# qiskit-community/adapt-aqc

Hardware: AMD Instinct MI355X
Metric: overlap+gradient evals/sec, 50-qubit MPS chi=64, 1/2/4/8 MI355X (higher is better)
Workload: dtype c128

## Files before the change

### adaptaqc_amd/_lib.py

```python
import atexit
import ctypes
import os
import threading

import numpy as np

_HERE = os.path.dirname(os.path.abspath(__file__))
LIB_PATH = os.environ.get("AQC_LIB") or os.path.join(_HERE, "libaqchip.so")

OP_DTYPE = np.dtype(
    [("nq", "<i4"), ("q0", "<i4"), ("q1", "<i4"), ("flags", "<i4"), ("m", "<f8", (32,))], align=True
)
assert OP_DTYPE.itemsize == 272
OP_KRAUS1 = 1
OP_MEASURE1 = 2
OP_KRAUS2 = 3

EXPORTS = (
    "aqc_last_error", "aqc_version", "aqc_init", "aqc_finalize", "aqc_timing_enable",
    "aqc_timing_query", "aqc_timing_reset",
    "aqc_sv_create", "aqc_sv_destroy", "aqc_sv_reset", "aqc_sv_copy", "aqc_sv_apply", "aqc_sv_plan",
    "aqc_sv_amp0", "aqc_sv_z_all", "aqc_sv_get", "aqc_sv_set",
    "aqc_mps_create", "aqc_mps_destroy", "aqc_mps_set_truncation", "aqc_mps_set_vidal",
    "aqc_mps_get_vidal", "aqc_mps_get_dims", "aqc_mps_copy", "aqc_mps_copy_batch", "aqc_mps_apply",
    "aqc_mps_apply_batch", "aqc_mps_apply_sort_batch", "aqc_mps_apply_sort_batch_async", "aqc_mps_apply_batch_async", "aqc_mps_check_batch", "aqc_mps_sort", "aqc_mps_sort_batch", "aqc_mps_overlap_zero",
    "aqc_mps_overlap_zero_batch", "aqc_mps_dot", "aqc_mps_z_all", "aqc_mps_amps_hw1", "aqc_mps_z_all_batch", "aqc_mps_z_sum_batch", "aqc_mps_zero_hw1_batch",
    "aqc_mps_amps_hw1_batch",
    "aqc_pair_grads", "aqc_pair_grads_batch", "aqc_argmax_scaled", "aqc_argmax_scaled_batch", "aqc_mps_jacobi_stats",
    "aqc_mps_set_jacobi_tol", "aqc_mps_set_jacobi_stop", "aqc_mps_set_fused_chain", "aqc_mps_chain_ticks", "aqc_svd_debug",
    "aqc_sv_pair_rdms", "aqc_mps_pair_rdms", "aqc_mps_pair_rdms_batch", "aqc_entanglement_measures",
    "aqc_sv_transition", "aqc_mps_product_fit", "aqc_mps_set_svd_path", "aqc_svd_gram_ticks", "aqc_bj_ticks",
    "aqc_sweep_set_chain_mode", "aqc_stream_join", "aqc_stream_wait", "aqc_svd_gram_stats", "aqc_env_ticks",
    "aqc_comm_unique_id", "aqc_comm_init", "aqc_comm_destroy", "aqc_comm_rank", "aqc_allgather_f64",
    "aqc_allgather_f64_host", "aqc_allreduce_max_f64", "aqc_svd_gram_big_stats", "aqc_svd_gram_big_ticks",
    "aqc_gb_set_spin_limit", "aqc_gb_set_tail", "aqc_gb_set_stages", "aqc_debug_hog", "aqc_pool_stats",
    "aqc_scratch_stats", "aqc_mps_set_chain_epilogue", "aqc_mps_get_chain_epilogue", "aqc_mps_chain_epilogue_stats",
    "aqc_env_fallbacks", "aqc_env_set_single", "aqc_env_set_spin_limit",
    "aqc_sv_sample", "aqc_mps_sample", "aqc_sample_uniforms", "aqc_sv_traj_sample",
    "aqc_sv_traj_pair_tomo", "aqc_sv_traj_pauli_counts", "aqc_mps_traj_sample", "aqc_mps_traj_plan", "aqc_mps_traj_set_batch",
    "aqc_mps_traj_pair_tomo", "aqc_mps_traj_tomo_plan", "aqc_mps_traj_set_readout_batch",
    "aqc_sv_pauli_expect", "aqc_mps_pauli_expect", "aqc_mps_pauli_expect_batch",
    "aqc_pair_tomo_probs", "aqc_concurrence_bound_probs", "aqc_multinomial_counts", "aqc_tomo_fit",
)


class AqcError(RuntimeError):
    pass


_lock = threading.Lock()
_lib = None
_initialised_device = None

_P = ctypes.c_void_p
_I = ctypes.c_int
_D = ctypes.c_double
_DP = ctypes.POINTER(ctypes.c_double)
_IP = ctypes.POINTER(ctypes.c_int)

_SIGS = {
    "aqc_last_error": ([], ctypes.c_char_p),
    "aqc_version": ([], _I),
    "aqc_init": ([_I], _I),
    "aqc_finalize": ([], _I),
    "aqc_timing_enable": ([_I], _I),
    "aqc_timing_query": ([ctypes.c_char_p, _DP, ctypes.POINTER(ctypes.c_int64), _DP, _DP], _I),
    "aqc_timing_reset": ([], _I),
    "aqc_sv_create": ([_I, ctypes.POINTER(_P)], _I),
    "aqc_sv_destroy": ([_P], _I),
    "aqc_sv_reset": ([_P], _I),
    "aqc_sv_copy": ([_P, _P], _I),
    "aqc_sv_apply": ([_P, _P, _I], _I),
    "aqc_sv_plan": ([_I, _P, _I, _P], _I),
    "aqc_sv_amp0": ([_P, _DP, _DP], _I),
    "aqc_sv_z_all": ([_P, _DP], _I),
    "aqc_sv_get": ([_P, _P], _I),
    "aqc_sv_set": ([_P, _P], _I),
    "aqc_mps_create": ([_I, _I, _D, _I, ctypes.POINTER(_P)], _I),
    "aqc_mps_destroy": ([_P], _I),
    "aqc_mps_set_truncation": ([_P, _D, _I], _I),
    "aqc_mps_set_vidal": ([_P, _P, _P, _P], _I),
    "aqc_mps_get_vidal": ([_P, _P, _P, _P], _I),
    "aqc_mps_get_dims": ([_P, _P], _I),
    "aqc_mps_copy": ([_P, _P], _I),
    "aqc_mps_copy_batch": ([_P, _P, _I], _I),
    "aqc_mps_apply": ([_P, _P, _I], _I),
    "aqc_mps_apply_batch": ([_P, _I, _P, _P], _I),
    "aqc_mps_apply_sort_batch": ([_P, _I, _P, _P], _I),
    "aqc_mps_apply_sort_batch_async": ([_P, _I, _P, _P], _I),
    "aqc_mps_apply_batch_async": ([_P, _I, _P, _P], _I),
    "aqc_mps_check_batch": ([_P, _I], _I),
    "aqc_mps_sort": ([_P], _I),
    "aqc_mps_sort_batch": ([_P, _I], _I),
    "aqc_mps_overlap_zero": ([_P, _DP, _DP], _I),
    "aqc_mps_overlap_zero_batch": ([_P, _I, _P], _I),
    "aqc_mps_dot": ([_P, _P, _DP, _DP], _I),
    "aqc_mps_z_all": ([_P, _P], _I),
    "aqc_mps_amps_hw1": ([_P, _P], _I),
    "aqc_mps_z_all_batch": ([_P, _I, _P], _I),
    "aqc_mps_z_sum_batch": ([_P, _P, _I, _P], _I),
    "aqc_mps_zero_hw1_batch": ([_P, _P, _I, _P, _P], _I),
    "aqc_mps_amps_hw1_batch": ([_P, _I, _P], _I),
    "aqc_pair_grads": ([_P, _P, _P, _I, _P, _P, _P, _I, _P, _I], _I),
    "aqc_pair_grads_batch": ([_P, _I, _P, _P, _I, _P, _P, _P, _I, _P, _I], _I),
    "aqc_argmax_scaled": ([_P, _P, _I, _I, _IP], _I),
    "aqc_argmax_scaled_batch": ([_P, _I, _P, _I, _I, _P], _I),
    "aqc_mps_jacobi_stats": ([_P, _IP], _I),
    "aqc_mps_set_jacobi_tol": ([_D], _I),
    "aqc_mps_set_jacobi_stop": ([_D], _I),
    "aqc_mps_set_fused_chain": ([_I], _I),
    "aqc_mps_chain_ticks": ([_P], _I),
    "aqc_mps_set_chain_epilogue": ([_I], _I),
    "aqc_mps_get_chain_epilogue": ([], _I),
    "aqc_mps_chain_epilogue_stats": ([_P], _I),
    "aqc_svd_debug": ([_P, _I, _I, _I, _I, _P, _P, _P, _P], _I),
    "aqc_sv_pair_rdms": ([_P, _P, _I, _P], _I),
    "aqc_mps_pair_rdms": ([_P, _P, _I, _P], _I),
    "aqc_mps_pair_rdms_batch": ([_P, _I, _P, _I, _P, _I], _I),
    "aqc_entanglement_measures": ([_P, _I, _I, _P, _I], _I),
    "aqc_sv_transition": ([_P, _P, _I, _P], _I),
    "aqc_mps_product_fit": ([_P, _P, _I, _I, _I, _D, _DP, _IP], _I),
    "aqc_mps_set_svd_path": ([_I, _I], _I),
    "aqc_svd_gram_ticks": ([_P], _I),
    "aqc_bj_ticks": ([_P], _I),
    "aqc_sweep_set_chain_mode": ([_I], _I),
    "aqc_stream_join": ([_P], _I),
    "aqc_stream_wait": ([_P], _I),
    "aqc_svd_gram_stats": ([_P], _I),
    "aqc_env_ticks": ([_P], _I),
    "aqc_comm_unique_id": ([ctypes.c_char_p], _I),
    "aqc_comm_init": ([ctypes.c_char_p, _I, _I, ctypes.POINTER(_P)], _I),
    "aqc_comm_destroy": ([_P], _I),
    "aqc_comm_rank": ([_P, _IP, _IP], _I),
    "aqc_allgather_f64": ([_P, _P, _P, ctypes.c_size_t], _I),
    "aqc_allgather_f64_host": ([_P, _P, _P, ctypes.c_size_t], _I),
    "aqc_allreduce_max_f64": ([_P, _DP], _I),
    "aqc_svd_gram_big_stats": ([_P], _I),
    "aqc_svd_gram_big_ticks": ([_P], _I),
    "aqc_gb_set_spin_limit": ([_D], _I),
    "aqc_env_fallbacks": ([ctypes.POINTER(ctypes.c_longlong)], _I),
    "aqc_env_set_single": ([_I], _I),
    "aqc_env_set_spin_limit": ([_D], _I),
    "aqc_gb_set_tail": ([_I], _I),
    "aqc_gb_set_stages": ([_I], _I),
    "aqc_debug_hog": ([_I, _D], _I),
    "aqc_pool_stats": ([_P], _I),
    "aqc_scratch_stats": ([_P], _I),
    "aqc_sv_sample": ([_P, _I, ctypes.c_uint64, ctypes.c_uint64, _P, _P], _I),
    "aqc_mps_sample": ([_P, _I, ctypes.c_uint64, ctypes.c_uint64, _P, _P], _I),
    "aqc_sample_uniforms": ([ctypes.c_uint64, ctypes.c_uint64, _I, _I, _P], _I),
    "aqc_sv_traj_sample": ([_I, _P, _I, _I, ctypes.c_uint64, ctypes.c_uint64, _P, _P, _P], _I),
    "aqc_sv_traj_pair_tomo": ([_I, _P, _I, _P, _I, _P, _I, ctypes.c_uint64, ctypes.c_uint64, _P, _P, _P], _I),
    "aqc_sv_traj_pauli_counts": ([_I, _P, _I, _P, _I, _P, _I, ctypes.c_uint64, ctypes.c_uint64, _P, _P, _P, _P], _I),
    "aqc_mps_traj_sample": ([_I, _I, _D, _I, _P, _I, _I, ctypes.c_uint64, ctypes.c_uint64, _P, _P, _P], _I),
    "aqc_mps_traj_plan": ([_I, _P, _I, _P, _P, _I], _I),
    "aqc_mps_traj_set_batch": ([_I], _I),
    "aqc_mps_traj_pair_tomo": ([_I, _I, _D, _I, _P, _I, _P, _I, _P, _I, ctypes.c_uint64, ctypes.c_uint64, _P, _P, _P], _I),
    "aqc_mps_traj_tomo_plan": ([_I, _P, _I, _P, _P, _I], _I),
    "aqc_mps_traj_set_readout_batch": ([_I], _I),
    "aqc_sv_pauli_expect": ([_P, _P, _P, _I, _P], _I),
    "aqc_mps_pauli_expect": ([_P, _P, _I, _P], _I),
    "aqc_mps_pauli_expect_batch": ([_P, _I, _P, _I, _P], _I),
    "aqc_pair_tomo_probs": ([_P, _I, _P, _I], _I),
    "aqc_concurrence_bound_probs": ([_P, _I, _P, _I], _I),
    "aqc_multinomial_counts": ([_P, _I, _I, _I, ctypes.c_uint64, ctypes.c_uint64, _P, _P], _I),
    "aqc_tomo_fit": ([_P, _I, _P, _I], _I),
}


def load(path=LIB_PATH):
    global _lib
    with _lock:
        if _lib is not None:
            return _lib
        if not os.path.exists(path):
            raise AqcError(
                f"HIP library not found at {path}; build it with `python -c 'import __graft_entry__ as g; g.build()'`"
            )
        try:
            import torch
        except ImportError:
            pass
        lib = ctypes.CDLL(path)
        missing = []
        for name, (args, res) in _SIGS.items():
            f = getattr(lib, name, None)
            if f is None:
                missing.append(name)
                continue
            f.argtypes = args
            f.restype = res
        if missing and not os.environ.get("AQC_LIB"):
            raise AqcError(f"{path} lacks entry points {missing}: rebuild it (make -C adaptaqc_amd/csrc)")
        _lib = lib
        return lib

# ... 91 lines not shown
```

### adaptaqc_amd/csrc/mps.hip

```cpp
#include <algorithm>
#include <cmath>
#include <chrono>
#include <cstring>
#include <atomic>
#include <cstdlib>
#include <mutex>
#include <thread>
#include <unordered_set>

#include "aqc_gemm.h"
#include "mps_internal.h"

using aqc::cplx;

namespace aqc {

namespace {
std::mutex g_mps_stream_mu;
hipStream_t g_mps_streams[64] = {nullptr};
void release_mps_streams() {
  std::lock_guard<std::mutex> lk(g_mps_stream_mu);
  for (auto& s : g_mps_streams)
    if (s) (void)hipStreamDestroy(s), s = nullptr;
}
}

hipStream_t mps_stream() {
  int dev = 0;
  hipGetDevice(&dev);
  std::lock_guard<std::mutex> lk(g_mps_stream_mu);
  if (!g_mps_streams[dev]) {
    hipStreamCreateWithFlags(&g_mps_streams[dev], hipStreamNonBlocking);
    note_device(dev);
    on_finalize(release_mps_streams);
  }
  return g_mps_streams[dev];
}

hipStream_t mps_stream_if_any(int dev) {
  if (dev < 0 || dev >= 64) return nullptr;
  std::lock_guard<std::mutex> lk(g_mps_stream_mu);
  return g_mps_streams[dev];
}

StagingRing& staging_ring() {
  static PerDevice<StagingRing> rings;
  return rings.here();
}

}

namespace {

using aqc::fresh_tid;
using aqc::StagingLease;
using aqc::wave_sum_d;

constexpr int kT = 256;
constexpr double kChop = 1e-16;
constexpr int kMaxSweeps = 60;
double g_jacobi_tol_factor = 1.0;
constexpr double kDefaultTinyT = 1e-6;
constexpr double kStopCos = 3e-13;
constexpr int kStopCosSweeps = 30;
double g_jacobi_tiny_t = kDefaultTinyT;
constexpr double kJacobiNoise = 0.0;
bool g_fused_chain = true;
int g_chain_epilogue = [] {
  const char* e = std::getenv("AQC_CHAIN_EPILOGUE");
  const int v = e ? std::atoi(e) : 3;
  return v >= 0 && v <= 3 ? v : 3;
}();
int g_chain_min_states = 32;
constexpr int kChainLdsBytes = 4 * (int)sizeof(aqc::GemmLds);

struct OneSiteJob {
  cplx* g;
  const int* dims;
  int cap;
  int pad;
  cplx u[4];
};

using aqc::TwoSiteJob;
using aqc::kMaxCap;
using aqc::kSigMax;
using aqc::kSigTail;
using aqc::kSigLen;

__global__ void k_mps_zero(cplx* gam, double* lam, int* dims, int n, int cap) {
  const size_t ss = (size_t)2 * cap * cap;
  for (int i = blockIdx.x * blockDim.x + threadIdx.x; i < n; i += gridDim.x * blockDim.x) {
    gam[(size_t)i * ss] = aqc::cmk(1.0, 0.0);
  }
  for (int b = blockIdx.x * blockDim.x + threadIdx.x; b <= n; b += gridDim.x * blockDim.x) {
    lam[(size_t)b * cap] = 1.0;
    dims[b] = 1;
  }
}

__global__ __launch_bounds__(kT) void k_1q(const OneSiteJob* __restrict__ jobs) {
  const OneSiteJob& j = jobs[blockIdx.y];
  const int cl = j.dims[0], cr = j.dims[1];
  const int cap = j.cap;
  const size_t half = (size_t)cap * cap;
  for (int e = blockIdx.x * kT + threadIdx.x; e < cl * cr; e += gridDim.x * kT) {
    const int l = e / cr, r = e % cr;
    const size_t o = (size_t)l * cap + r;
    const cplx a0 = aqc::ldg(j.g + o), a1 = aqc::ldg(j.g + half + o);
    aqc::stg(j.g + o, aqc::cfma(j.u[1], a1, aqc::cmul(j.u[0], a0)));
    aqc::stg(j.g + half + o, aqc::cfma(j.u[3], a1, aqc::cmul(j.u[2], a0)));
  }
}

__global__ __launch_bounds__(kT) void k_theta(const TwoSiteJob* __restrict__ jobs, int nj) {
  int jb, tile;
  if (!aqc::xcd_job_block(nj, jb, tile)) return;
  const TwoSiteJob& j = jobs[jb];
  const int chl = j.dims[0], chm = j.dims[1], chr = j.dims[2];
  const int cap = j.cap;
  const int tiles_r = (cap + 15) / 16;
  const int l0 = (tile / tiles_r) * 16, r0 = (tile % tiles_r) * 16;
  if (l0 >= chl || r0 >= chr) return;
  __shared__ cplx As[2][16][17];
  __shared__ cplx Bs[2][16][17];
  const int ty = threadIdx.x / 16, tx = threadIdx.x % 16;
  const int l = l0 + ty, r = r0 + tx;
  const size_t half = (size_t)cap * cap;
  cplx acc[4];
#pragma unroll
  for (int i = 0; i < 4; ++i) acc[i] = aqc::cmk(0, 0);
  const double lll = l < chl ? j.ll[l] : 0.0;
  const double lrr = r < chr ? j.lr[r] : 0.0;
  for (int m0 = 0; m0 < chm; m0 += 16) {
    const int ma = m0 + tx, mb = m0 + ty;
#pragma unroll
    for (int s = 0; s < 2; ++s) {
      cplx a = aqc::cmk(0, 0), b = aqc::cmk(0, 0);
      if (l < chl && ma < chm) a = aqc::cscale(j.gp[s * half + (size_t)l * cap + ma], lll * j.lm[ma]);
      if (mb < chm && r < chr) b = aqc::cscale(j.gq[s * half + (size_t)mb * cap + r], lrr);
      As[s][ty][tx] = a;
      Bs[s][ty][tx] = b;
    }
    __syncthreads();
#pragma unroll 4
    for (int mm = 0; mm < 16; ++mm) {
      const cplx a0 = As[0][ty][mm], a1 = As[1][ty][mm];
      const cplx b0 = Bs[0][mm][tx], b1 = Bs[1][mm][tx];
      acc[0] = aqc::cfma(a0, b0, acc[0]);
      acc[1] = aqc::cfma(a0, b1, acc[1]);
      acc[2] = aqc::cfma(a1, b0, acc[2]);
      acc[3] = aqc::cfma(a1, b1, acc[3]);
    }
    __syncthreads();
// ... 806 lines not shown
  const double* llp = j.ll;
  const double* lmp = j.lm;
  const double* lrp = j.lr;
  asm volatile("" : "+s"(gp), "+s"(gq), "+s"(llp), "+s"(lmp), "+s"(lrp));
  __shared__ cplx sG[16];
  if (tid < 16) sG[tid] = aqc::ldg(j.G + tid);
  const int as1 = tid >> 9, al = (tid >> 3) & 63, am = tid & 7;
  const int bs2 = tid >> 9, bm = (tid >> 6) & 7, br = tid & 63;
  auto fetch = [&](int m0, cplx& a, cplx& b) {
    const int ma = m0 + am, mb = m0 + bm;
    a = (al < chl && ma < chm) ? aqc::cscale(aqc::ldg(gp + as1 * half + (size_t)al * cap + ma), aqc::ldg(llp + al) * aqc::ldg(lmp + ma))
                               : aqc::cmk(0, 0);
    b = (mb < chm && br < chr) ? aqc::cscale(aqc::ldg(gq + bs2 * half + (size_t)mb * cap + br), aqc::ldg(lrp + br)) : aqc::cmk(0, 0);
  };
  auto stash = [&](int buf, cplx a, cplx b) {
    cplx* base = xbuf + buf * kThetaMfmaBuf;
    base[(as1 * 64 + al) * kThetaMfmaAP + am] = a;
    base[2 * 64 * kThetaMfmaAP + (bs2 * 8 + bm) * kThetaMfmaBP + br] = b;
  };
  aqc::d4_t cr[2][2], ci[2][2];
#pragma unroll
  for (int s1 = 0; s1 < 2; ++s1)
#pragma unroll
    for (int s2 = 0; s2 < 2; ++s2) cr[s1][s2] = aqc::d4_t{0, 0, 0, 0}, ci[s1][s2] = aqc::d4_t{0, 0, 0, 0};
  const int nch = (chm + 7) >> 3;
  {
    cplx a, b;
    fetch(0, a, b);
    stash(0, a, b);
  }
  __syncthreads();
  for (int c = 0; c < nch; ++c) {
    const bool more = c + 1 < nch;
    cplx na = aqc::cmk(0, 0), nb = aqc::cmk(0, 0);
    if (more) fetch(8 * (c + 1), na, nb);
    if (active) {
      const cplx* base = xbuf + (c & 1) * kThetaMfmaBuf;
      const cplx* As = base;
      const cplx* Bs = base + 2 * 64 * kThetaMfmaAP;
#pragma unroll
      for (int ks = 0; ks < 2; ++ks) {
        const int mm = 4 * ks + lk;
        cplx x[2], y[2];
#pragma unroll
        for (int s = 0; s < 2; ++s) {
          x[s] = Bs[(s * 8 + mm) * kThetaMfmaBP + r0 + li];
          y[s] = As[(s * 64 + l0 + li) * kThetaMfmaAP + mm];
        }
#pragma unroll
        for (int s1 = 0; s1 < 2; ++s1)
#pragma unroll
          for (int s2 = 0; s2 < 2; ++s2) {
            cr[s1][s2] = __builtin_amdgcn_mfma_f64_16x16x4f64(x[s2].x, y[s1].x, cr[s1][s2], 0, 0, 0);
            cr[s1][s2] = __builtin_amdgcn_mfma_f64_16x16x4f64(-x[s2].y, y[s1].y, cr[s1][s2], 0, 0, 0);
            ci[s1][s2] = __builtin_amdgcn_mfma_f64_16x16x4f64(x[s2].x, y[s1].y, ci[s1][s2], 0, 0, 0);
            ci[s1][s2] = __builtin_amdgcn_mfma_f64_16x16x4f64(x[s2].y, y[s1].x, ci[s1][s2], 0, 0, 0);
          }
      }
    }
    if (more) stash((c + 1) & 1, na, nb);
    __syncthreads();
  }
  if (active) {
    const int l = l0 + li;
#pragma unroll
    for (int q = 0; q < 4; ++q) {
      const int r = r0 + lk + 4 * q;
      if (l < chl && r < chr) {
        const cplx p0 = aqc::cmk(cr[0][0][q], ci[0][0][q]), p1 = aqc::cmk(cr[0][1][q], ci[0][1][q]);
        const cplx p2 = aqc::cmk(cr[1][0][q], ci[1][0][q]), p3 = aqc::cmk(cr[1][1][q], ci[1][1][q]);
#pragma unroll
        for (int o = 0; o < 4; ++o) {
          cplx v = aqc::cmul(sG[o * 4 + 0], p0);
          v = aqc::cfma(sG[o * 4 + 1], p1, v);
          v = aqc::cfma(sG[o * 4 + 2], p2, v);
          v = aqc::cfma(sG[o * 4 + 3], p3, v);
          aqc::stg(j.theta + (size_t)((o & 1) * chr + r) * M + (o >> 1) * chl + l, v);
        }
      }
    }
  }
}

__device__ __noinline__ void chain_jacobi_fallback(const TwoSiteJob& j) { jacobi_reg_body<128, 8, 16>(j); }
__device__ __forceinline__ int chain_jacobi(const TwoSiteJob& j, int epi) {
  if (j.gram) {
    const int g = gram_svd_body(j, epi);
    if (g == 1) return 0;
    if (g > 2) return g - 2;
    __syncthreads();
    if (g == 2 && gram_certified(j)) return 0;
  }
  chain_jacobi_fallback(j);
  return 0;
}
__device__ __forceinline__ void chain_rank(const TwoSiteJob& j) { rank_body<1024, 128>(j); }
__device__ __forceinline__ void split_gemm_chain(const TwoSiteJob& j, int tid) {
  extern __shared__ double2 xbuf[];
  const int sg = tid >> 8, lt = tid & 255, blk = sg >> 1, h = sg & 1;
  const int chl = j.dims[0], k = j.dims[1], chr = j.dims[2];
  const int M = 2 * chl, N = 2 * chr;
  const bool tr = (M < N) != (j.qr != 0);
  const int L = tr ? N : M;
  const int cap = j.cap;
  const size_t half = (size_t)cap * cap;
  const double* ss = j.sig + kSigMax;
  const int rows = tr ? M : k, cols = tr ? k : N;
  const int r0 = tr ? 64 * blk : 0, c0 = tr ? 0 : 64 * blk;
  const bool active = r0 < rows && c0 < cols;
  const int mb = active ? min(64, rows - r0) : 64, nb = active ? min(64, cols - c0) : 64;
  const int kh = ((L + 1) / 2 + 15) & ~15, klo = h * kh;
  const cplx* W = j.work;
  const int* perm = j.perm;
  const cplx* th = j.theta;
  aqc::GemmLds& lds = reinterpret_cast<aqc::GemmLds*>(xbuf)[sg];
  aqc::d4_t cr[2][2], ci[2][2];
  if (!tr) {
    aqc::block_cgemm_tile<true, true, false>(
        mb, nb, kh, 0, 0,
        [&](int kk, int R) {
          return klo + R < L ? aqc::cconj(aqc::ldg(W + (size_t)perm[r0 + kk] * L + klo + R)) : aqc::cmk(0, 0);
        },
        [&](int R, int c) { return klo + R < L ? aqc::ldg(th + (size_t)(c0 + c) * M + klo + R) : aqc::cmk(0, 0); }, lds, lt,
        active, cr, ci);
  } else {
    aqc::block_cgemm_tile<false, true, false>(
        mb, nb, kh, 0, 0,
        [&](int R, int c) { return klo + c < L ? aqc::ldg(th + (size_t)(klo + c) * M + r0 + R) : aqc::cmk(0, 0); },
        [&](int c, int kk) { return klo + c < L ? aqc::ldg(W + (size_t)perm[c0 + kk] * L + klo + c) : aqc::cmk(0, 0); }, lds,
        lt, active, cr, ci);
  }
  cplx* part = xbuf + blk * (64 * 64);
  const int wave = lt >> 6, lane = lt & 63;
  const int wr = (wave >> 1) * 32, wc = (wave & 1) * 32, li = lane & 15, lk = lane >> 4;
  if (active && h == 1) {
#pragma unroll
    for (int r = 0; r < 2; ++r)
#pragma unroll
      for (int c = 0; c < 2; ++c)
#pragma unroll
        for (int q = 0; q < 4; ++q)
          part[(wr + 16 * r + lk + 4 * q) * 64 + wc + 16 * c + li] = aqc::cmk(cr[r][c][q], ci[r][c][q]);
  }
  __syncthreads();
  if (active && h == 0) {
#pragma unroll
    for (int r = 0; r < 2; ++r)
#pragma unroll
      for (int c = 0; c < 2; ++c)
#pragma unroll
        for (int q = 0; q < 4; ++q) {
          const int i = wr + 16 * r + lk + 4 * q, jj = wc + 16 * c + li;
          if (i < mb && jj < nb) {
            const cplx o = part[i * 64 + jj];
            const cplx v = aqc::cmk(cr[r][c][q] + o.x, ci[r][c][q] + o.y);
            if (!tr) {
              const int kq = r0 + i, cc = c0 + jj, s2 = cc / chr, rr = cc % chr;
              const double sk = aqc::ldg(ss + kq), d = sk * sk * aqc::ldg(j.lr + rr);
              aqc::stg(j.gq + s2 * half + (size_t)kq * cap + rr, d != 0.0 ? aqc::cscale(v, 1.0 / d) : aqc::cmk(0, 0));
            } else {
              const int Rr = r0 + i, kq = c0 + jj, s1 = Rr / chl, l = Rr % chl;
              const double sk = aqc::ldg(ss + kq), d = sk * sk * aqc::ldg(j.ll + l);
              aqc::stg(j.gp + s1 * half + (size_t)l * cap + kq, d != 0.0 ? aqc::cscale(v, 1.0 / d) : aqc::cmk(0, 0));
            }
          }
        }
  }
}
template <bool TR>
__device__ __forceinline__ void split_lds_body(const TwoSiteJob& j, int tid) {
  extern __shared__ double2 xbuf[];
  const cplx* Vl = xbuf;
  const double* rcp = reinterpret_cast<const double*>(xbuf + kVlElems);
  const int chl = j.dims[0], k = j.dims[1], chr = j.dims[2];
  const int M = 2 * chl, N = 2 * chr;
  const int C = TR ? N : M;
  const int cap = j.cap;
  const size_t half = (size_t)cap * cap;
  if (TR) {
    for (int e = tid; e < N * k; e += 1024) {
      const int cc = e % N, kk = e / N;
      const int s2 = cc >= chr, r = cc - s2 * chr;
      const double f = rcp[kVlRcpSig + kk] != 0.0 ? rcp[kVlRcpLr + r] : 0.0;
      const cplx v = Vl[kVlPos(cc, kk)];
      aqc::stg(j.gq + s2 * half + (size_t)kk * cap + r, aqc::cmk(v.x * f, -v.y * f));
    }
  } else {
    for (int e = tid; e < M * k; e += 1024) {
      const int kk = e % k, R = e / k;
      const int s1 = R >= chl, l = R - s1 * chl;
      const double f = rcp[kVlRcpSig + kk] != 0.0 ? rcp[kVlRcpLl + l] : 0.0;
      const cplx v = Vl[kVlPos(R, kk)];
      aqc::stg(j.gp + s1 * half + (size_t)l * cap + kk, aqc::cmk(v.x * f, v.y * f));
    }
  }
  const int wave = __builtin_amdgcn_readfirstlane(tid >> 6), lane = tid & 63;
  const int li = lane & 15, lk = lane >> 4;
  const int rt = wave >> 1, ct = 2 * (wave & 1);
  const int outer = TR ? M : N;
  if (16 * rt >= outer) return;
  const int m = 16 * rt + li;
  const bool mok = m < outer;
  const cplx* tp = j.theta + (TR ? (size_t)lk * M + m : (size_t)m * M + lk);
  const size_t ts = TR ? (size_t)4 * M : 4;
  auto ldt = [&](int s) { return (mok && 4 * s + lk < C) ? aqc::ldg(tp + s * ts) : aqc::cmk(0, 0); };
  aqc::d4_t p1[2], p2[2], p3[2];
#pragma unroll
  for (int u = 0; u < 2; ++u) p1[u] = p2[u] = p3[u] = aqc::d4_t{0, 0, 0, 0};
  auto kstep = [&](int s, cplx t) {
    const int row = 4 * s + lk;
    const double tsum = t.x + t.y;
#pragma unroll
    for (int u = 0; u < 2; ++u) {
      const cplx v = Vl[kVlPos(row, 16 * (ct + u) + li)];
      if (TR) {
        p1[u] = __builtin_amdgcn_mfma_f64_16x16x4f64(t.x, v.x, p1[u], 0, 0, 0);
        p2[u] = __builtin_amdgcn_mfma_f64_16x16x4f64(t.y, v.y, p2[u], 0, 0, 0);
        p3[u] = __builtin_amdgcn_mfma_f64_16x16x4f64(tsum, v.x + v.y, p3[u], 0, 0, 0);
      } else {
        p1[u] = __builtin_amdgcn_mfma_f64_16x16x4f64(v.x, t.x, p1[u], 0, 0, 0);
        p2[u] = __builtin_amdgcn_mfma_f64_16x16x4f64(v.y, t.y, p2[u], 0, 0, 0);
        p3[u] = __builtin_amdgcn_mfma_f64_16x16x4f64(v.x - v.y, tsum, p3[u], 0, 0, 0);
      }
    }
  };
  const int nks = (C + 3) >> 2;
  cplx t0 = ldt(0), t1 = ldt(1);
  for (int s = 0; s < nks; s += 2) {
    const cplx n0 = ldt(s + 2), n1 = ldt(s + 3);
    kstep(s, t0);
    if (s + 1 < nks) kstep(s + 1, t1);
    t0 = n0;
    t1 = n1;
  }
#pragma unroll
  for (int u = 0; u < 2; ++u) {
#pragma unroll
    for (int q = 0; q < 4; ++q) {
      const double re = TR ? p1[u][q] - p2[u][q] : p1[u][q] + p2[u][q];
      const double im = TR ? p3[u][q] - p1[u][q] - p2[u][q] : p3[u][q] - p1[u][q] + p2[u][q];
      const int kq = 16 * (ct + u) + (TR ? li : lk + 4 * q);
      const int o = 16 * rt + (TR ? lk + 4 * q : li);
      if (kq < k && o < outer) {
        const int ch = TR ? chl : chr;
        const int s = o >= ch, b = o - s * ch;
        const double f1 = rcp[kVlRcpSig + kq], f2 = rcp[(TR ? kVlRcpLl : kVlRcpLr) + b];
        const cplx g = aqc::cmk(re * f1 * f2, im * f1 * f2);
        if (TR) aqc::stg(j.gp + s * half + (size_t)b * cap + kq, g);
        else aqc::stg(j.gq + s * half + (size_t)kq * cap + b, g);
      }
    }
  }
}
__device__ __forceinline__ void split_lds_chain(const TwoSiteJob& j, int tid) {
  const bool tr = 2 * j.dims[0] >= 2 * j.dims[2];
  if (tr) split_lds_body<true>(j, tid);
  else split_lds_body<false>(j, tid);
}
__device__ __forceinline__ void chain_split(const TwoSiteJob& j, int done) {
  const int tid = fresh_tid();
  if (done == 3) {
    split_lds_chain(j, tid);
    return;
  }
  if (done != 2) split_copy_body(j, tid, 1024);
  split_gemm_chain(j, tid);
}

__global__ __launch_bounds__(1024) void k_chain(const ChainJob* __restrict__ chains, const TwoSiteJob* __restrict__ two,
                                                const OneSiteJob* __restrict__ one, int epi) {
  const ChainJob& c = chains[blockIdx.x];
  const int tid = fresh_tid();
  __shared__ unsigned long long tk[6];
  if (tid == 0) tk[0] = tk[1] = tk[2] = tk[3] = tk[4] = tk[5] = 0;
  auto tick = [&](int ph) {
    if (tid == 0) {
      const unsigned long long t = __builtin_amdgcn_s_memtime();
      if (ph >= 0) tk[ph] += t - tk[5];
      tk[5] = t;
    }
  };
  tick(-1);
  for (int o = 0; o < c.nops; ++o) {
    const int code = __builtin_amdgcn_readfirstlane(c.ops[o]);
    if (code < 0) {
      one_site_body(one[-code - 1], tid, 1024);
      __syncthreads();
      tick(4);
      continue;
    }
    const TwoSiteJob& j = two[code];
#if AQC_THETA_MFMA
    chain_theta_mfma(j);
#else
    chain_theta(j);
#endif
    __syncthreads();
    tick(0);
    const int done = __builtin_amdgcn_readfirstlane(chain_jacobi(j, epi));
    __syncthreads();
    tick(1);
    if (done == 0) chain_rank(j);
    __syncthreads();
    tick(2);
    chain_split(j, done);
    __syncthreads();
    tick(3);
  }
  if (tid == 0)
    for (int ph = 0; ph < 5; ++ph) atomicAdd(&g_chain_ticks[ph], tk[ph]);
}

using aqc::DevOp;
using aqc::Scheduler;
using aqc::KrausJob;
using aqc::TrajCtx;
using aqc::run_waves;

template <class F>
void parallel_states(int ns, F&& f) {
  static const int kThreads = [] {
    const char* e = std::getenv("AQC_HOST_THREADS");
    const int v = e ? std::atoi(e) : 1;
    return v < 1 ? 1 : (v > 64 ? 64 : v);
  }();
  const int nt = std::min(kThreads, ns / 32);
  if (nt <= 1) {
    for (int s = 0; s < ns; ++s) f(s);
    return;
  }
  std::vector<std::thread> th;
  th.reserve(nt - 1);
  for (int t = 1; t < nt; ++t)
    th.emplace_back([&f, t, nt, ns] {
      for (int s = t; s < ns; s += nt) f(s);
    });
  for (int s = 0; s < ns; s += nt) f(s);
  for (auto& x : th) x.join();
}

bool distinct_handles(aqc_mps_t* hs, int ns) {
  std::unordered_set<const void*> seen;
  seen.reserve(2 * ns);
  for (int s = 0; s < ns; ++s)
    if (!seen.insert(hs[s]).second) return false;
  return true;
}

int validate_ops(aqc_mps_t h, const aqc_op_t* ops, int nops) {
  for (int i = 0; i < nops; ++i) {
    const aqc_op_t& o = ops[i];
    AQC_REQUIRE(o.nq == 1 || o.nq == 2, "aqc_mps_apply: only 1- and 2-qubit ops are supported");
    AQC_REQUIRE(o.q0 >= 0 && o.q0 < h->d.n, "aqc_mps_apply: qubit index out of range");
    if (o.nq == 2) AQC_REQUIRE(o.q1 >= 0 && o.q1 < h->d.n && o.q1 != o.q0, "aqc_mps_apply: bad second qubit");
  }
  return AQC_OK;
}

void schedule(aqc_mps_t h, const aqc_op_t* ops, int nops, bool sort_after, std::vector<DevOp>& out) {
  Scheduler s(h->d.n, h->order, h->loc, out);
  for (int i = 0; i < nops; ++i) {
    if (ops[i].nq == 1) s.one(ops[i].q0, ops[i].m);
    else s.two(ops[i].q0, ops[i].q1, ops[i].m);
  }
  s.flush();
  if (sort_after) s.sort();
}

TwoSiteJob make_two(aqc_mps_t h, const DevOp& op, int slot = 0) {
  TwoSiteJob j;
  std::memset(&j, 0, sizeof(j));
  const int p = op.p;
  j.gp = h->d.site(p);
  j.gq = h->d.site(p + 1);
  j.ll = h->d.bond(p);
  j.lm = h->d.bond(p + 1);
// ... 49 lines not shown
    AQC_HIP_CHECK(hipMemsetAsync(sl.sig, 0, kSigLen * sizeof(double), aqc::mps_stream()));
    h->slots.push_back(sl);
  }
  return AQC_OK;
}

std::vector<std::vector<const DevOp*>> level_ops(const std::vector<DevOp>& ops, int n) {
  std::vector<int> last(n + 1, -1);
  std::vector<std::vector<const DevOp*>> lv;
  for (const DevOp& op : ops) {
    int l;
    if (op.kind == 2) {
      l = std::max(last[op.p], last[op.p + 1]) + 1;
      last[op.p] = last[op.p + 1] = l;
    } else {
      l = last[op.p] + 1;
      last[op.p] = l;
    }
    if ((int)lv.size() <= l) lv.resize(l + 1);
    lv[l].push_back(&op);
  }
  return lv;
}

int run_chains(aqc_mps_t* hs, int ns, std::vector<std::vector<DevOp>>& lists, int cap_max) {
  hipStream_t st = aqc::mps_stream();
  std::vector<size_t> off2(ns + 1, 0), off1(ns + 1, 0), offc(ns + 1, 0);
  for (int s = 0; s < ns; ++s) {
    size_t n2 = 0;
    for (const DevOp& op : lists[s]) n2 += op.kind == 2;
    off2[s + 1] = off2[s] + n2;
    off1[s + 1] = off1[s] + (lists[s].size() - n2);
    offc[s + 1] = offc[s] + lists[s].size();
  }
  const size_t n_two = off2[ns], n_one = off1[ns], n_codes = offc[ns];
  if (n_codes == 0) return AQC_OK;
  std::vector<int> order(ns);
  for (int s = 0; s < ns; ++s) order[s] = s;
  std::stable_sort(order.begin(), order.end(),
                   [&](int a, int b) { return lists[a].size() > lists[b].size(); });
  auto al = [](size_t x) { return (x + 255) & ~(size_t)255; };
  const size_t o_two = 0, o_one = al(o_two + n_two * sizeof(TwoSiteJob));
  const size_t o_codes = al(o_one + n_one * sizeof(OneSiteJob));
  const size_t o_chain = al(o_codes + n_codes * sizeof(int));
  const size_t total = o_chain + (size_t)ns * sizeof(ChainJob);
  StagingLease lease(st);
  if (lease.rc() != AQC_OK) return lease.rc();
  aqc::DevScratch& sg = lease.buf();
  int rc = lease.ensure(total);
  if (rc != AQC_OK) return rc;
  char* hb = sg.host;
  char* db = sg.dev;
  TwoSiteJob* h2 = (TwoSiteJob*)(hb + o_two);
  OneSiteJob* h1 = (OneSiteJob*)(hb + o_one);
  int* hcode = (int*)(hb + o_codes);
  parallel_states(ns, [&](int s) {
    size_t i2 = off2[s], i1 = off1[s], ic = offc[s];
    for (const DevOp& op : lists[s]) {
      if (op.kind == 2) {
        h2[i2] = make_two(hs[s], op, 0);
        h2[i2].qr = 1;
        hcode[ic++] = (int)i2++;
        std::vector<int>& ub = hs[s]->ub;
        int nb = std::min(2 * std::min(ub[op.p], ub[op.p + 2]), hs[s]->d.cap);
        if (hs[s]->max_chi > 0) nb = std::min(nb, hs[s]->max_chi);
        ub[op.p + 1] = std::max(nb, 1);
      } else {
        h1[i1] = make_one(hs[s], op);
        hcode[ic++] = -(int)(++i1);
      }
    }
  });
  ChainJob* hc = (ChainJob*)(hb + o_chain);
  for (int k = 0; k < ns; ++k) {
    const int s = order[k];
    hc[k].ops = (const int*)(db + o_codes) + offc[s];
    hc[k].nops = (int)lists[s].size();
    hc[k].pad = 0;
  }
  if (int e = aqc::upload_async(sg.dev, sg.host, total, st)) return e;
  const double c = cap_max, nj = (double)n_two;
  aqc::KernelTimer::begin(st, "mps_chain", nj * 8.0 * c * c * 16, nj * (84.0 * 8.0 + 64.0) * c * c * c);
  hipLaunchKernelGGL(k_chain, dim3(ns), dim3(1024), kChainLds, st, (const ChainJob*)(db + o_chain),
                     (const TwoSiteJob*)(db + o_two), (const OneSiteJob*)(db + o_one), g_chain_epilogue);
  aqc::KernelTimer::end(st);
  AQC_CHECK_LAUNCH();
  return AQC_OK;
}

KrausJob make_kraus(aqc_mps_t h, const DevOp& op, int shot) {
  KrausJob j;
  std::memset(&j, 0, sizeof(j));
  j.g = h->d.site(op.p);
  j.ll = h->d.bond(op.p);
  j.lr = h->d.bond(op.p + 1);
  j.dims = h->d.dims + op.p;
  j.cap = h->d.cap;
  j.nk = op.nk;
  j.slot = op.slot;
  j.meas = op.meas;
  j.shot = shot;
  std::memcpy(j.K, op.m, sizeof(j.K));
  for (int k = 0; k < op.nk; ++k) {
    const cplx* K = op.m + 4 * k;
    j.w[4 * k] = K[0].x * K[0].x + K[0].y * K[0].y + K[2].x * K[2].x + K[2].y * K[2].y;
    j.w[4 * k + 1] = K[1].x * K[1].x + K[1].y * K[1].y + K[3].x * K[3].x + K[3].y * K[3].y;
    j.w[4 * k + 2] = K[0].x * K[1].x + K[0].y * K[1].y + K[2].x * K[3].x + K[2].y * K[3].y;
    j.w[4 * k + 3] = K[0].x * K[1].y - K[0].y * K[1].x + K[2].x * K[3].y - K[2].y * K[3].x;
  }
  return j;
}

}

int aqc::run_waves(aqc_mps_t* hs, int ns, std::vector<std::vector<DevOp>>& lists, const TrajCtx* ctx) {
  bool kraus = false;
  for (int s = 0; s < ns; ++s) {
    int lo = 1 << 30, hi = -1;
    for (const DevOp& op : lists[s]) {
      lo = std::min(lo, op.p);
      hi = std::max(hi, op.kind == 2 ? op.p + 1 : op.p);
      kraus |= op.kind == 3;
    }
    if (hi >= 0) hs[s]->changed(lo, hi);
  }
  if (kraus && !ctx) {
    aqc::set_error("run_waves: Kraus rows without a trajectory context");
    return AQC_ERR_ARG;
  }
  if (!kraus) {
    int cap_max = 0;
    for (int s = 0; s < ns; ++s) cap_max = std::max(cap_max, hs[s]->d.cap);
    if (g_fused_chain && ns >= g_chain_min_states && 2 * cap_max > 64 && 2 * cap_max <= 128)
      return run_chains(hs, ns, lists, cap_max);
  }
  hipStream_t st = aqc::mps_stream();
  std::vector<std::vector<std::vector<const DevOp*>>> lv(ns);
  size_t maxlen = 0;
  for (int s = 0; s < ns; ++s) {
    lv[s] = level_ops(lists[s], hs[s]->d.n);
    maxlen = std::max(maxlen, lv[s].size());
    int width = 1;
    for (auto& w : lv[s]) {
      int k = 0;
      for (const DevOp* op : w) k += op->kind == 2;
      width = std::max(width, k);
    }
    int rc = ensure_slots(hs[s], width);
    if (rc != AQC_OK) return rc;
  }
  if (maxlen == 0) return AQC_OK;
  std::vector<TwoSiteJob> two;
  std::vector<OneSiteJob> one;
  std::vector<KrausJob> kr;
  std::vector<std::pair<size_t, size_t>> two_rng(maxlen), one_rng(maxlen), kr_rng(maxlen);
  int cap_max = 0;
  for (int s = 0; s < ns; ++s) cap_max = std::max(cap_max, hs[s]->d.cap);
  struct ClassRange {
    int cls;
    size_t first, count;
  };
  std::vector<std::vector<ClassRange>> wave_cls(maxlen);
  auto class_of = [&](int side) {
    if (2 * cap_max <= 128) return 2 * cap_max;
    if (side <= 32) return 32;
    if (side <= 64) return 64;
    if (side <= 128) return 128;
// ... 346 lines not shown
  const int L = std::max(m, n), C = std::min(m, n);
  const int Lw = j.qr ? C : L;
  AQC_HIP_CHECK(hipMemcpyAsync(w_out, wk, (size_t)C * Lw * sizeof(cplx), hipMemcpyDeviceToHost, st));
  AQC_HIP_CHECK(hipMemcpyAsync(sig_out, sg, (size_t)C * sizeof(double), hipMemcpyDeviceToHost, st));
  if (perm_out) AQC_HIP_CHECK(hipMemcpyAsync(perm_out, pm, (size_t)C * sizeof(int), hipMemcpyDeviceToHost, st));
  AQC_HIP_CHECK(hipMemcpyAsync(hd, fl, 4 * sizeof(int), hipMemcpyDeviceToHost, st));
  AQC_HIP_CHECK(hipStreamSynchronize(st));
  *sweeps = hd[2];
  AQC_HIP_CHECK(hipFree(buf));
  return AQC_OK;
}

int aqc_mps_jacobi_stats(aqc_mps_t h, int* max_sweeps) {
  AQC_REQUIRE(h && max_sweeps, "aqc_mps_jacobi_stats: null argument");
  hipStream_t st = aqc::mps_stream();
  int f[3] = {0, 0, 0};
  AQC_HIP_CHECK(hipMemcpyAsync(f, h->d.flags, sizeof(f), hipMemcpyDeviceToHost, st));
  AQC_HIP_CHECK(hipStreamSynchronize(st));
  *max_sweeps = f[2];
  int z = 0;
  AQC_HIP_CHECK(hipMemcpy(h->d.flags + 2, &z, sizeof(int), hipMemcpyHostToDevice));
  return AQC_OK;
}

int aqc_mps_set_jacobi_tol(double factor) {
  AQC_REQUIRE(factor > 0, "aqc_mps_set_jacobi_tol: factor must be positive");
  g_jacobi_tol_factor = factor;
  return AQC_OK;
}

int aqc_svd_gram_ticks(double* out) {
  AQC_REQUIRE(out, "aqc_svd_gram_ticks: null argument");
  unsigned long long t[12];
  AQC_HIP_CHECK(hipMemcpyFromSymbol(t, HIP_SYMBOL(g_gram_ticks), sizeof(t)));
  for (int i = 0; i < 12; ++i) out[i] = (double)t[i];
  unsigned long long z[12] = {0, 0, 0, 0, 0, 0, 0, 0, 0, 0, 0, 0};
  AQC_HIP_CHECK(hipMemcpyToSymbol(HIP_SYMBOL(g_gram_ticks), z, sizeof(z)));
  return AQC_OK;
}

int aqc_svd_gram_stats(double* out) {
  AQC_REQUIRE(out, "aqc_svd_gram_stats: null argument");
  unsigned long long t[6];
  AQC_HIP_CHECK(hipMemcpyFromSymbol(t, HIP_SYMBOL(g_gram_stats), sizeof(t)));
  for (int i = 0; i < 6; ++i) out[i] = (double)t[i];
  unsigned long long z[6] = {0, 0, 0, 0, 0, 0};
  AQC_HIP_CHECK(hipMemcpyToSymbol(HIP_SYMBOL(g_gram_stats), z, sizeof(z)));
  return AQC_OK;
}

int aqc_mps_set_svd_path(int gram, int debug_max_chi) {
  AQC_REQUIRE(gram >= 0 && gram <= 1, "aqc_mps_set_svd_path: gram must be 0 or 1");
  g_svd_gram = gram;
  g_debug_max_chi = debug_max_chi;
  return AQC_OK;
}


int aqc_mps_set_jacobi_stop(double tiny_t) {
  AQC_REQUIRE(tiny_t < 1e-3, "aqc_mps_set_jacobi_stop: tiny_t must be < 1e-3 (<= 0 restores the default)");
  g_jacobi_tiny_t = tiny_t > 0 ? tiny_t : kDefaultTinyT;
  return AQC_OK;
}

int aqc_mps_chain_ticks(double* out) {
  AQC_REQUIRE(out, "aqc_mps_chain_ticks: null argument");
  unsigned long long t[5] = {0, 0, 0, 0, 0};
  AQC_HIP_CHECK(hipStreamSynchronize(aqc::mps_stream()));
  AQC_HIP_CHECK(hipMemcpyFromSymbol(t, HIP_SYMBOL(g_chain_ticks), sizeof(t)));
  const unsigned long long z[5] = {0, 0, 0, 0, 0};
  AQC_HIP_CHECK(hipMemcpyToSymbol(HIP_SYMBOL(g_chain_ticks), z, sizeof(z)));
  for (int i = 0; i < 5; ++i) out[i] = (double)t[i];
  return AQC_OK;
}

int aqc_mps_set_chain_epilogue(int mode) {
  AQC_REQUIRE(mode >= 0 && mode <= 3, "aqc_mps_set_chain_epilogue: 0, 1, 2 or 3");
  g_chain_epilogue = mode;
  return AQC_OK;
}

int aqc_mps_get_chain_epilogue(void) { return g_chain_epilogue; }

int aqc_mps_chain_epilogue_stats(double* out) {
  AQC_REQUIRE(out, "aqc_mps_chain_epilogue_stats: null argument");
  unsigned long long t[2] = {0, 0};
  AQC_HIP_CHECK(hipStreamSynchronize(aqc::mps_stream()));
  AQC_HIP_CHECK(hipMemcpyFromSymbol(t, HIP_SYMBOL(g_epi_stats), sizeof(t)));
  const unsigned long long z[2] = {0, 0};
  AQC_HIP_CHECK(hipMemcpyToSymbol(HIP_SYMBOL(g_epi_stats), z, sizeof(z)));
  for (int i = 0; i < 2; ++i) out[i] = (double)t[i];
  return AQC_OK;
}

int aqc_mps_set_fused_chain(int on) {
  AQC_REQUIRE(on >= 0 && on <= 2, "aqc_mps_set_fused_chain: 0, 1 or 2");
  g_fused_chain = on != 0;
  g_chain_min_states = on == 2 ? 1 : 32;
  return AQC_OK;
}


int aqc_mps_set_truncation(aqc_mps_t h, double threshold, int max_chi) {
  AQC_REQUIRE(h, "aqc_mps_set_truncation: null handle");
  h->thr = threshold;
  h->max_chi = max_chi;
  return AQC_OK;
}

int aqc_mps_set_vidal(aqc_mps_t h, const int* dims, const double* gammas, const double* lambdas) {
  AQC_REQUIRE(h && dims && gammas && lambdas, "aqc_mps_set_vidal: null argument");
  const int n = h->d.n, cap = h->d.cap;
  AQC_REQUIRE(dims[0] == 1 && dims[n] == 1, "aqc_mps_set_vidal: dims[0] and dims[n] must be 1");
  for (int b = 0; b <= n; ++b) {
    if (dims[b] < 1 || dims[b] > cap) {
      aqc::set_error("aqc_mps_set_vidal: bond dimension exceeds chi_cap");
      return AQC_ERR_ARG;
    }
  }
  std::vector<cplx> g((size_t)n * 2 * cap * cap, aqc::cmk(0, 0));
  std::vector<double> l((size_t)(n + 1) * cap, 0.0);
  size_t off = 0;
  for (int i = 0; i < n; ++i)
    for (int s = 0; s < 2; ++s)
      for (int a = 0; a < dims[i]; ++a)
        for (int b = 0; b < dims[i + 1]; ++b, ++off)
          g[(size_t)i * 2 * cap * cap + (size_t)s * cap * cap + (size_t)a * cap + b] =
              aqc::cmk(gammas[2 * off], gammas[2 * off + 1]);
  l[0] = 1.0;
  l[(size_t)n * cap] = 1.0;
  size_t lo = 0;
  for (int b = 1; b < n; ++b)
    for (int k = 0; k < dims[b]; ++k) l[(size_t)b * cap + k] = lambdas[lo++];
  hipStream_t st = aqc::mps_stream();
  AQC_HIP_CHECK(hipStreamSynchronize(st));
  AQC_HIP_CHECK(hipMemcpy(h->d.gam, g.data(), g.size() * sizeof(cplx), hipMemcpyHostToDevice));
  AQC_HIP_CHECK(hipMemcpy(h->d.lam, l.data(), l.size() * sizeof(double), hipMemcpyHostToDevice));
  AQC_HIP_CHECK(hipMemcpy(h->d.dims, dims, (n + 1) * sizeof(int), hipMemcpyHostToDevice));
  for (int i = 0; i < n; ++i) h->order[i] = h->loc[i] = i;
  h->ub.assign(dims, dims + n + 1);
  h->changed_all();
  return AQC_OK;
}

int aqc_mps_get_dims(aqc_mps_t h, int* dims) {
  AQC_REQUIRE(h && dims, "aqc_mps_get_dims: null argument");
  hipStream_t st = aqc::mps_stream();
  AQC_HIP_CHECK(hipMemcpyAsync(dims, h->d.dims, (h->d.n + 1) * sizeof(int), hipMemcpyDeviceToHost, st));
  AQC_HIP_CHECK(hipStreamSynchronize(st));
  h->ub.assign(dims, dims + h->d.n + 1);
  return AQC_OK;
}

int aqc_mps_sort(aqc_mps_t h) {
  AQC_REQUIRE(h, "aqc_mps_sort: null handle");
  if (is_sorted_order(h)) return AQC_OK;
  int rc = do_sort(&h, 1);
  if (rc != AQC_OK) return rc;
  return check_flags(h);
}

int aqc_mps_sort_batch(aqc_mps_t* hs, int ns) {
  AQC_REQUIRE(hs && ns >= 0, "aqc_mps_sort_batch: bad arguments");
  int moved = 0;
  int rc = do_sort(hs, ns, &moved);
  if (rc != AQC_OK) return rc;
// ... 214 lines not shown
```

### include/aqc_hip_diag.h

```cpp
#ifndef AQC_HIP_DIAG_H
#define AQC_HIP_DIAG_H

#include "aqc_hip.h"

#ifdef __cplusplus
extern "C" {
#endif

int aqc_mps_jacobi_stats(aqc_mps_t h, int* max_sweeps);
int aqc_mps_set_jacobi_tol(double factor);
int aqc_mps_set_jacobi_stop(double tiny_t);
int aqc_mps_set_svd_path(int gram, int debug_max_chi);
int aqc_svd_gram_ticks(double* out);
int aqc_svd_gram_stats(double* out);
int aqc_env_ticks(double* out);
int aqc_env_fallbacks(long long* out);
int aqc_env_set_single(int on);
int aqc_env_set_spin_limit(double us);
int aqc_bj_ticks(double* out);
int aqc_svd_gram_big_stats(double* out);
int aqc_svd_gram_big_ticks(double* out);
int aqc_gb_set_spin_limit(double us);
int aqc_gb_set_tail(int on);
int aqc_gb_set_stages(int n);
int aqc_debug_hog(int nblocks, double ms);
int aqc_pool_stats(double* out);
int aqc_scratch_stats(double* out);
int aqc_mps_set_fused_chain(int on);
int aqc_mps_set_chain_epilogue(int mode);
int aqc_mps_get_chain_epilogue(void);
int aqc_mps_chain_epilogue_stats(double* out);
int aqc_mps_chain_ticks(double* out);
int aqc_svd_debug(const double* theta, int m, int n, int variant, int stop_after_qr, double* w_out,
                  double* sig_out, int* perm_out, int* sweeps);
int aqc_sweep_set_chain_mode(int mode);
int aqc_sample_uniforms(uint64_t seed, uint64_t run, int nshots, int nper, double* out);
#ifdef __cplusplus
}
#endif
#endif
```

Before: 8.588 million.

## Add specialized cap-64 theta contraction with staged LDS and software-pipelined loads

Adds a specialized theta-building path for two-site jobs whose bond dims are multiples of 16/8 at cap 64. It stages the right site, scaled by its singular values, plus the gate in LDS, then streams the left site with double-buffered loads around MFMA f64 steps. A second change software-pipelines the K loop of another contraction by four steps when its dimensions are 16-aligned. The goal is to hide global-load latency and skip the generic theta path's overhead, at the cost of more code and register pressure. A runtime/env switch (default on) selects the new path.

Result: no change. 8.584 million (-0.1%).

```diff
diff --git a/adaptaqc_amd/_lib.py b/adaptaqc_amd/_lib.py
--- a/adaptaqc_amd/_lib.py
+++ b/adaptaqc_amd/_lib.py
@@ -35,6 +35,7 @@
     "aqc_allgather_f64_host", "aqc_allreduce_max_f64", "aqc_svd_gram_big_stats", "aqc_svd_gram_big_ticks",
     "aqc_gb_set_spin_limit", "aqc_gb_set_tail", "aqc_gb_set_stages", "aqc_debug_hog", "aqc_pool_stats",
     "aqc_scratch_stats", "aqc_mps_set_chain_epilogue", "aqc_mps_get_chain_epilogue", "aqc_mps_chain_epilogue_stats",
+    "aqc_mps_set_chain_theta", "aqc_mps_get_chain_theta",
     "aqc_env_fallbacks", "aqc_env_set_single", "aqc_env_set_spin_limit",
     "aqc_sv_sample", "aqc_mps_sample", "aqc_sample_uniforms", "aqc_sv_traj_sample",
     "aqc_sv_traj_pair_tomo", "aqc_sv_traj_pauli_counts", "aqc_mps_traj_sample", "aqc_mps_traj_plan", "aqc_mps_traj_set_batch",
@@ -112,6 +113,8 @@
     "aqc_mps_chain_ticks": ([_P], _I),
     "aqc_mps_set_chain_epilogue": ([_I], _I),
     "aqc_mps_get_chain_epilogue": ([], _I),
+    "aqc_mps_set_chain_theta": ([_I], _I),
+    "aqc_mps_get_chain_theta": ([], _I),
     "aqc_mps_chain_epilogue_stats": ([_P], _I),
     "aqc_svd_debug": ([_P, _I, _I, _I, _I, _P, _P, _P, _P], _I),
     "aqc_sv_pair_rdms": ([_P, _P, _I, _P], _I),
diff --git a/adaptaqc_amd/csrc/mps.hip b/adaptaqc_amd/csrc/mps.hip
--- a/adaptaqc_amd/csrc/mps.hip
+++ b/adaptaqc_amd/csrc/mps.hip
@@ -70,6 +70,11 @@
   const char* e = std::getenv("AQC_CHAIN_EPILOGUE");
   const int v = e ? std::atoi(e) : 3;
   return v >= 0 && v <= 3 ? v : 3;
+}();
+int g_chain_theta = [] {
+  const char* e = std::getenv("AQC_CHAIN_THETA");
+  const int v = e ? std::atoi(e) : 1;
+  return v >= 0 && v <= 1 ? v : 1;
 }();
 int g_chain_min_states = 32;
 constexpr int kChainLdsBytes = 4 * (int)sizeof(aqc::GemmLds);
@@ -1042,6 +1047,118 @@
   }
 }
 
+constexpr int kThBElems = 2 * 64 * 64;
+constexpr int kThGOff = kThBElems;
+constexpr int kThLmOff = kThBElems + 16;
+static_assert((kThLmOff + 32) * 16 <= kChainLdsBytes, "theta's staged site exceeds the chain's LDS");
+__device__ __forceinline__ int kThPos(int s2, int m, int r) { return (s2 * 64 + m) * 64 + r; }
+__device__ __forceinline__ bool chain_theta_full(const TwoSiteJob& j) {
+  return ((j.dims[0] | j.dims[2]) & 15) == 0 && (j.dims[1] & 7) == 0 && j.dims[0] > 0 && j.dims[1] > 0 && j.dims[2] > 0 &&
+         j.cap == 64;
+}
+__device__ __noinline__ void chain_theta_direct(const TwoSiteJob& j, const cplx* gp, const cplx* gq, const double* llp,
+                                                const double* lmp, const double* lrp, cplx* theta, int chl, int chm,
+                                                int chr) {
+  extern __shared__ double2 xbuf[];
+  cplx* Bt = xbuf;
+  cplx* sG = xbuf + kThGOff;
+  double* lml = reinterpret_cast<double*>(xbuf + kThLmOff);
+  const int tid = fresh_tid(), wave = tid >> 6, lane = tid & 63, li = lane & 15, lk = lane >> 4;
+  gp = uniform_ptr(gp), gq = uniform_ptr(gq), llp = uniform_ptr(llp), lmp = uniform_ptr(lmp), lrp = uniform_ptr(lrp);
+  theta = uniform_ptr(theta);
+  chl = __builtin_amdgcn_readfirstlane(chl), chm = __builtin_amdgcn_readfirstlane(chm);
+  chr = __builtin_amdgcn_readfirstlane(chr);
+  constexpr int cap = 64;
+  constexpr size_t half = (size_t)cap * cap;
+  const int M = 2 * chl;
+  const int r0 = 16 * (wave >> 2), l0 = 16 * (wave & 3);
+  const bool active = r0 < chr && l0 < chl;
+  const int l = min(l0 + li, chl - 1);
+  const cplx* ap = gp + (size_t)l * cap + lk;
+  auto lda = [&](int s, cplx (&t)[2]) {
+    t[0] = aqc::ldg(ap + 4 * s);
+    t[1] = aqc::ldg(ap + half + 4 * s);
+  };
+  const int sr = tid & 63, sm = tid >> 6;
+  const int rc = min(sr, chr - 1);
+  cplx stg_v[2][4];
+#pragma unroll
+  for (int s2 = 0; s2 < 2; ++s2)
+#pragma unroll
+    for (int i = 0; i < 4; ++i) stg_v[s2][i] = aqc::ldg(gq + s2 * half + (size_t)min(sm + 16 * i, chm - 1) * cap + rc);
+  const double lrv = aqc::ldg(lrp + rc);
+  const double lmv = aqc::ldg(lmp + min(sr, chm - 1));
+  const cplx gv = aqc::ldg(j.G + (tid & 15));
+  const double llv = aqc::ldg(llp + l);
+  cplx t0[2], t1[2];
+  __builtin_amdgcn_sched_barrier(0);
+  lda(0, t0);
+  __builtin_amdgcn_sched_barrier(0);
+  lda(1, t1);
+  __builtin_amdgcn_sched_barrier(0);
+#pragma unroll
+  for (int s2 = 0; s2 < 2; ++s2)
+#pragma unroll
+    for (int i = 0; i < 4; ++i) Bt[kThPos(s2, sm + 16 * i, sr)] = aqc::cscale(stg_v[s2][i], lrv);
+  sG[tid & 15] = gv;
+  lml[sr] = lmv;
+  __syncthreads();
+  if (!active) return;
+  aqc::d4_t cr[2][2], ci[2][2];
+#pragma unroll
+  for (int s1 = 0; s1 < 2; ++s1)
+#pragma unroll
+    for (int s2 = 0; s2 < 2; ++s2) cr[s1][s2] = aqc::d4_t{0, 0, 0, 0}, ci[s1][s2] = aqc::d4_t{0, 0, 0, 0};
+  const cplx* xp = Bt + kThPos(0, lk, r0 + li);
+  auto mfmas = [&](const cplx (&x)[2], const cplx (&y)[2]) {
+#pragma unroll
+    for (int s1 = 0; s1 < 2; ++s1)
+#pragma unroll
+      for (int s2 = 0; s2 < 2; ++s2) {
+        cr[s1][s2] = __builtin_amdgcn_mfma_f64_16x16x4f64(x[s2].x, y[s1].x, cr[s1][s2], 0, 0, 0);
+        cr[s1][s2] = __builtin_amdgcn_mfma_f64_16x16x4f64(-x[s2].y, y[s1].y, cr[s1][s2], 0, 0, 0);
+        ci[s1][s2] = __builtin_amdgcn_mfma_f64_16x16x4f64(x[s2].x, y[s1].y, ci[s1][s2], 0, 0, 0);
+        ci[s1][s2] = __builtin_amdgcn_mfma_f64_16x16x4f64(x[s2].y, y[s1].x, ci[s1][s2], 0, 0, 0);
+      }
+  };
+  auto kstep = [&](int s, const cplx(&t)[2]) {
+    const double w = llv * lml[4 * s + lk];
+    cplx x[2], y[2];
+#pragma unroll
+    for (int s2 = 0; s2 < 2; ++s2) x[s2] = xp[kThPos(s2, 4 * s, 0)];
+#pragma unroll
+    for (int s1 = 0; s1 < 2; ++s1) y[s1] = aqc::cscale(t[s1], w);
+    mfmas(x, y);
+  };
+  const int nks = chm >> 2;
+  int s = 0;
+  for (; s + 2 < nks; s += 2) {
+    kstep(s, t0);
+    __builtin_amdgcn_sched_barrier(0);
+    lda(s + 2, t0);
+    kstep(s + 1, t1);
+    __builtin_amdgcn_sched_barrier(0);
+    lda(s + 3, t1);
+  }
+  kstep(s, t0);
+  kstep(s + 1, t1);
+  const int lo = l0 + li;
+#pragma unroll
+  for (int q = 0; q < 4; ++q) {
+    const int r = r0 + lk + 4 * q;
+    const cplx p0 = aqc::cmk(cr[0][0][q], ci[0][0][q]), p1 = aqc::cmk(cr[0][1][q], ci[0][1][q]);
+    const cplx p2 = aqc::cmk(cr[1][0][q], ci[1][0][q]), p3 = aqc::cmk(cr[1][1][q], ci[1][1][q]);
+#pragma unroll
+    for (int o = 0; o < 4; ++o) {
+      cplx v = aqc::cmul(sG[o * 4 + 0], p0);
+      v = aqc::cfma(sG[o * 4 + 1], p1, v);
+      v = aqc::cfma(sG[o * 4 + 2], p2, v);
+      v = aqc::cfma(sG[o * 4 + 3], p3, v);
+      aqc::stg(theta + (size_t)((o & 1) * chr + r) * M + (o >> 1) * chl + lo, v);
+    }
+  }
+}
+
 __device__ __noinline__ void chain_jacobi_fallback(const TwoSiteJob& j) { jacobi_reg_body<128, 8, 16>(j); }
 __device__ __forceinline__ int chain_jacobi(const TwoSiteJob& j, int epi) {
   if (j.gram) {
@@ -1185,13 +1302,37 @@
     }
   };
   const int nks = (C + 3) >> 2;
-  cplx t0 = ldt(0), t1 = ldt(1);
-  for (int s = 0; s < nks; s += 2) {
-    const cplx n0 = ldt(s + 2), n1 = ldt(s + 3);
+  if ((outer & 15) == 0 && (C & 15) == 0) {
+    auto ldf = [&](int s) { return aqc::ldg(tp + s * ts); };
+    cplx t0 = ldf(0), t1 = ldf(1);
+    int s = 0;
+    for (; s + 4 < nks; s += 4) {
+      cplx n0 = ldf(s + 2), n1 = ldf(s + 3);
+      __builtin_amdgcn_sched_barrier(0);
+      kstep(s, t0);
+      kstep(s + 1, t1);
+      __builtin_amdgcn_sched_barrier(0);
+      t0 = ldf(s + 4), t1 = ldf(s + 5);
+      __builtin_amdgcn_sched_barrier(0);
+      kstep(s + 2, n0);
+      kstep(s + 3, n1);
+      __builtin_amdgcn_sched_barrier(0);
+    }
+    const cplx n0 = ldf(s + 2), n1 = ldf(s + 3);
+    __builtin_amdgcn_sched_barrier(0);
     kstep(s, t0);
-    if (s + 1 < nks) kstep(s + 1, t1);
-    t0 = n0;
-    t1 = n1;
+    kstep(s + 1, t1);
+    kstep(s + 2, n0);
+    kstep(s + 3, n1);
+  } else {
+    cplx t0 = ldt(0), t1 = ldt(1);
+    for (int s = 0; s < nks; s += 2) {
+      const cplx n0 = ldt(s + 2), n1 = ldt(s + 3);
+      kstep(s, t0);
+      if (s + 1 < nks) kstep(s + 1, t1);
+      t0 = n0;
+      t1 = n1;
+    }
   }
 #pragma unroll
   for (int u = 0; u < 2; ++u) {
@@ -1228,7 +1369,7 @@
 }
 
 __global__ __launch_bounds__(1024) void k_chain(const ChainJob* __restrict__ chains, const TwoSiteJob* __restrict__ two,
-                                                const OneSiteJob* __restrict__ one, int epi) {
+                                                const OneSiteJob* __restrict__ one, int epi, int th) {
   const ChainJob& c = chains[blockIdx.x];
   const int tid = fresh_tid();
   __shared__ unsigned long long tk[6];
@@ -1251,7 +1392,9 @@
     }
     const TwoSiteJob& j = two[code];
 #if AQC_THETA_MFMA
-    chain_theta_mfma(j);
+    if (th != 0 && chain_theta_full(j))
+      chain_theta_direct(j, j.gp, j.gq, j.ll, j.lm, j.lr, j.theta, j.dims[0], j.dims[1], j.dims[2]);
+    else chain_theta_mfma(j);
 #else
     chain_theta(j);
 #endif
@@ -1467,7 +1610,8 @@
   const double c = cap_max, nj = (double)n_two;
   aqc::KernelTimer::begin(st, "mps_chain", nj * 8.0 * c * c * 16, nj * (84.0 * 8.0 + 64.0) * c * c * c);
   hipLaunchKernelGGL(k_chain, dim3(ns), dim3(1024), kChainLds, st, (const ChainJob*)(db + o_chain),
-                     (const TwoSiteJob*)(db + o_two), (const OneSiteJob*)(db + o_one), g_chain_epilogue);
+                     (const TwoSiteJob*)(db + o_two), (const OneSiteJob*)(db + o_one), g_chain_epilogue,
+                     g_chain_theta);
   aqc::KernelTimer::end(st);
   AQC_CHECK_LAUNCH();
   return AQC_OK;
@@ -1980,6 +2124,14 @@
 
 int aqc_mps_get_chain_epilogue(void) { return g_chain_epilogue; }
 
+int aqc_mps_set_chain_theta(int mode) {
+  AQC_REQUIRE(mode >= 0 && mode <= 1, "aqc_mps_set_chain_theta: 0 or 1");
+  g_chain_theta = mode;
+  return AQC_OK;
+}
+
+int aqc_mps_get_chain_theta(void) { return g_chain_theta; }
+
 int aqc_mps_chain_epilogue_stats(double* out) {
   AQC_REQUIRE(out, "aqc_mps_chain_epilogue_stats: null argument");
   unsigned long long t[2] = {0, 0};
diff --git a/include/aqc_hip_diag.h b/include/aqc_hip_diag.h
--- a/include/aqc_hip_diag.h
+++ b/include/aqc_hip_diag.h
@@ -29,6 +29,8 @@
 int aqc_mps_set_fused_chain(int on);
 int aqc_mps_set_chain_epilogue(int mode);
 int aqc_mps_get_chain_epilogue(void);
+int aqc_mps_set_chain_theta(int mode);
+int aqc_mps_get_chain_theta(void);
 int aqc_mps_chain_epilogue_stats(double* out);
 int aqc_mps_chain_ticks(double* out);
 int aqc_svd_debug(const double* theta, int m, int n, int variant, int stop_after_qr, double* w_out,
```
